# akshilpatel/tile-match-gym

Measured on AMD Instinct MI355X. Metric: env-steps/sec (whole node), 65536×10×10 boards, at 1/2/4/8 MI355X, higher is better.
Workload: dtype int8; 1 GPU; c2: 65536 x 10x10 boards per GPU, 4 colours, no specials, num_moves=30, autoreset, 3 episode-phase blocks offset by 10 steps, the timed window opening on a block's reset step (phases + 4); boards_per_gpu=65536, rows=10, cols=10, colours=4, env_groups_per_gpu=3, phase_blocks=3, policy=uniform, api=raw, graph=False, parallelism=dp1 (independent env shards, no collective)

## Files before the change

### tile-match-gym_amd/csrc/tmg_board.hip

```cpp
#include <hip/hip_runtime.h>
#include <stdint.h>

#include "pcg64.h"

namespace tmg {

#define WSYNC() __syncthreads()

#ifndef TMG_LEAN128_WAVES
#define TMG_LEAN128_WAVES 8
#endif
constexpr int kLean128Waves = TMG_LEAN128_WAVES;
constexpr int kLean128GenericWaves = 7;
constexpr int kGen128Waves = 5;
#ifndef TMG_RESET512_WAVES
#define TMG_RESET512_WAVES 8
#endif
#ifndef TMG_RESET128_WAVES
#define TMG_RESET128_WAVES 8
#endif
constexpr int kReset512Waves = TMG_RESET512_WAVES;
constexpr int kReset128Waves = TMG_RESET128_WAVES;
constexpr int kC5StepWaves = 4;

#define WFENCE() __builtin_amdgcn_fence(__ATOMIC_SEQ_CST, "wavefront")

#ifndef TMG_SMEM_DECL
#define TMG_SMEM_DECL(name) extern __shared__ __align__(16) unsigned char name[]
#endif

enum : int { SP_COOKIE = 1, SP_VLASER = 2, SP_HLASER = 4, SP_BOMB = 8 };
enum : int { M_NORMAL = 0, M_VLASER = 1, M_HLASER = 2, M_BOMB = 3, M_COOKIE = 4 };
enum : int { FL_DONE = 1, FL_COMBO = 2, FL_SHUF = 4, FL_RESET = 8, FL_OVF = 0x40, FL_ERR = 0x80 };
enum : int { TIER_MAIN = 0, TIER_SPILL = 2 };
enum : uint32_t { ST_INTERNAL = 1, ST_OVERFLOW = 2, ST_CALLER = 4 };

constexpr int kMaxShuffles = 1 << 12;

constexpr int kSpillWaves = 16;
struct SpillQ {
    uint32_t count, done;
    unsigned long long total;
    int64_t cap;
    int64_t env[1];
};

#ifndef TMG_COVER
#define TMG_COVER 0
#endif
enum : int {
    CV_SB_LEAN = 0,
    CV_SB_NORMAL,
    CV_SB_LASER,
    CV_SB_PERP_BOMB,
    CV_SB_ROW_BOMB,
    CV_SB_CLOSURE,
    CV_SB_FALLBACK,
    CV_LDS_NORMAL,
    CV_LDS_LASER,
    CV_LDS_BOMB,
    CV_LDS_FALLBACK,
    CV_SERIAL_STEP,
    CV_SERIAL_ACT,
    CV_SERIAL_COOKIE,
    CV_COMBO,
    CV_SPILL,
    CV_SPILL_RUN,
    CV_SHUFFLE,
    CV_REJECT,
    CV_FAST,
    CV_SHUFFLE_GEN,
    CV_REJECT_GEN,
    CV_RP_PASSES,
    CV_RP_PERP,
    CV_RP_VLONG,
    CV_RP_WIDE,
    CV_RP_REJECT,
    CV_LANE_STEP,
    CV_LANE_SHUFFLE,
    CV_LANE_REDRAW,
    CV_LANE_REJECT,
    CV_LANE_REJECT_REDRAW,
    CV_COUNT = 32
};
#if TMG_COVER
#define COVER(site)                                                                                     \
    do {                                                                                                \
        if (lane == 0 && P.cover) atomicAdd(P.cover + (site), 1ULL);                                   \
    } while (0)
#define COVER_L0(site)                                                                                  \
    do {                                                                                                \
        if (P.cover) atomicAdd(P.cover + (site), 1ULL);                                                \
    } while (0)
#else
#define COVER(site) ((void)0)
#define COVER_L0(site) ((void)0)
#endif

struct Params {
    int R, C, N, A, W, k, smask, num_moves;
    uint32_t thr;
    uint32_t cmag, cm1mag;
    const uint64_t *jump;
    uint64_t sb_nl[2];
    uint64_t sb_nf[2];
    uint64_t sb_h[2];
    uint64_t sb_z;
    uint64_t sb_in[2], sb_u[2], sb_v[2];
    const uint64_t *sb_rows;
    uint32_t *status;
    void *oh;
    int oh_dtype, oh_ch, oh_nsel;
    uint32_t oh_sel;
    SpillQ *spill;
    void *spill_ws;
    unsigned long long *cover;
    uint8_t *vo_term;
    uint8_t *vo_mask;
    int64_t *vo_left;
    int8_t *vo_final;
    int32_t *vo_obs;
    int sample;
    int32_t pol_t;
    int64_t pol_first;
    uint64_t pol_key;
};

#ifndef TMG_KERNARG_PARAMS
#if defined(__HIP_DEVICE_COMPILE__)
#define TMG_KERNARG_PARAMS(p) (*(const Params *)__builtin_amdgcn_kernarg_segment_ptr())
#else
#define TMG_KERNARG_PARAMS(p) (p)
#endif
#endif

inline void build_sb_rows(int R, int C, uint64_t *tab) {
    for (int r = 0; r < R; r++) {
        uint64_t m[4] = {0, 0, 0, 0};
        for (int p = 0; p < (r + 1) * C && p < 128; p++) {
            if (p >= r * C) m[p & 1] |= 1ULL << (p >> 1);
            m[2 + (p & 1)] |= 1ULL << (p >> 1);
        }
        for (int i = 0; i < 4; i++) tab[r * 4 + i] = m[i];
    }
}

inline Params make_params(int R, int C, int k, int smask, int num_moves, const uint64_t *jump) {
    Params P;
    P.R = R; P.C = C; P.N = R * C;
    P.A = 2 * R * C - R - C;
    P.W = (P.A + 63) / 64;
    P.k = k; P.smask = smask; P.num_moves = num_moves;
    const uint32_t rng = (uint32_t)(k - 1), excl = rng + 1;
    P.thr = rng ? (UINT32_MAX - rng) % excl : 0u;
    P.cmag = ((1u << 20) + (uint32_t)C - 1) / (uint32_t)C;
    P.cm1mag = C > 1 ? ((1u << 20) + (uint32_t)C - 2) / (uint32_t)(C - 1) : 0u;
    P.jump = jump;
    for (int w = 0; w < 2; w++) P.sb_nl[w] = P.sb_nf[w] = P.sb_h[w] = P.sb_in[w] = P.sb_u[w] = P.sb_v[w] = 0;
    P.sb_z = 0;
    P.sb_rows = nullptr;
    P.status = nullptr;
    P.spill = nullptr;
    P.spill_ws = nullptr;
    P.cover = nullptr;
    P.oh = nullptr;
    P.oh_dtype = P.oh_ch = P.oh_nsel = 0;
    P.oh_sel = 0;
    P.vo_term = nullptr;
    P.vo_mask = nullptr;
    P.vo_left = nullptr;
    P.vo_final = nullptr;
    P.vo_obs = nullptr;
    P.sample = 0;
    P.pol_t = 0;
    P.pol_first = 0;
    P.pol_key = 0;
    if (P.N <= 128) {
        for (int p = 0; p < P.N; p++) {
            const int c = p % C, w = p & 1, b = p >> 1;
            P.sb_in[w] |= 1ULL << b;
            if (p >= C) P.sb_u[w] |= 1ULL << b;
            if (p >= 2 * C) P.sb_v[w] |= 1ULL << b;
            if (c <= C - 2) P.sb_nl[w] |= 1ULL << b;
            if (c >= 1) P.sb_nf[w] |= 1ULL << b;
            if (c <= C - 3) P.sb_h[w] |= 1ULL << b;
        }
        const int stride = (C & 1) ? C : C / 2;
        for (int b = 0; b < 64; b += stride) P.sb_z |= 1ULL << b;
    }
    return P;
}

__device__ __forceinline__ int div_c(const Params &P, int x) { return (int)(((uint32_t)x * P.cmag) >> 20); }
__device__ __forceinline__ int div_cm1(const Params &P, int x) { return (int)(((uint32_t)x * P.cm1mag) >> 20); }


__device__ __forceinline__ int64_t wg_env() {
    const int64_t per = gridDim.x >> 3;
    return (int64_t)(blockIdx.x & 7) * per + (blockIdx.x >> 3);
}

enum : int { SC_NACT = 0, SC_NNEW, SC_ERR, SC_NZ, SC_A, SC_B, SC_C, SC_D, SC_COUNT = 16 };

template <int MAXN_>
struct WsCore {
    static constexpr int MAXN = MAXN_;
    static constexpr int NP = MAXN / 64;
    static constexpr int MAXW = (2 * MAXN) / 64 + 2;
    uint64_t effw[MAXW];
    int32_t sc[SC_COUNT];
    static constexpr int PRE = MAXW * 8 + SC_COUNT * 4;
    int8_t lpad[PRE >= 128 ? 1 : 128 - PRE];
    alignas(4) int8_t brd[2 * MAXN];
    uint8_t mark[MAXN];
    alignas(8) int8_t trash[4 * 64];
    union alignas(16) {
        uint32_t draw[MAXN + 128];
        struct { int8_t tmp[2 * MAXN]; int16_t perm[MAXN]; } sh;
    } u;
};

template <int POOL_, int MLINES_, int MQ_, int MM_, int MPOOL_, int MSTK_>
struct ListStore {
    static constexpr int POOL = POOL_;
    static constexpr int MLINES = MLINES_;
    static constexpr int MQ = MQ_;
    static constexpr int MM = MM_;
    static constexpr int MPOOL = MPOOL_;
    static constexpr int MSTK = MSTK_;
    static constexpr int MV = 96;
    int16_t pool[POOL];
    int16_t ls[MLINES], ll[MLINES];
    int16_t q[MQ];
    int16_t mpool[MPOOL];
    int16_t ms[MM], mlen[MM];
    int8_t mname[MM], mcol[MM];
// ... 1731 lines not shown
            activate(r * C + c, 2, true);
            activate(r * C + c, 3, true);
        } else if ((t1 == 4 && t2 >= 2 && t2 <= 3) || (t2 == 4 && t1 >= 2 && t1 <= 3)) {
            clr(p1); clr(p2);
            int r = r1 < r2 ? r1 : r2, c = c1 < c2 ? c1 : c2;
            int a0 = r > 0 ? r - 1 : 0, a1 = r < R - 1 ? r + 1 : R - 1;
            int b0 = c > 0 ? c - 1 : 0, b1 = c < C - 1 ? c + 1 : C - 1;
            for (int i = a0; i <= a1; i++) activate(i * C + c, 3, true);
            for (int j = b0; j <= b1; j++) activate(r * C + j, 2, true);
        } else if (t1 == 4 && t2 == 4) {
            clr(p1); clr(p2);
            int r = r1 < r2 ? r1 : r2, c = c1 < c2 ? c1 : c2;
            int a0 = r > 1 ? r - 2 : 0, a1 = r < R - 2 ? r + 2 : R - 1;
            int b0 = c > 1 ? c - 2 : 0, b1 = c < C - 2 ? c + 2 : C - 1;
            for (int i = a0; i <= a1; i++)
                for (int j = b0; j <= b1; j++) {
                    int p = i * C + j, t = typ[p];
                    if (t == 1) clr(p);
                    else if (t != 0) activate(p, t, true);
                }
        }
    }
};


#include "tmg_sb.hip"

template <int MAXN, bool GEN, int SBNB, bool CODD, int TIER, class WS, class L>
__device__ __forceinline__ int board_move(const Params &P, WS &w, int lane, const LaneJump &J, Rng &g,
                          const Cells<MAXN / 64> &cl, int p1, int p2, int &flags, int &nn, int &na, int64_t e,
                          L *lists, bool clean) {
    const auto cells = [&]() {
        if constexpr (MAXN > 128) return cl;
        else return make_cells<MAXN / 64>(P, loop_lane(lane));
    };
    const int N = P.N;
    int lim = P.R - 1;
    if (clean) lim = min(P.R - 1, div_c(P, max(p1, p2)) + 2);
    int8_t *col = w.brd, *typ = w.brd + N;
    int elim = 0;
    if (lane == 0) {
        int8_t x = col[p1]; col[p1] = col[p2]; col[p2] = x;
        x = typ[p1]; typ[p1] = typ[p2]; typ[p2] = x;
        w.sc[SC_NACT] = 0; w.sc[SC_NNEW] = 0; w.sc[SC_ERR] = 0; w.sc[SC_A] = 0;
    }
    WSYNC();
    const int t1 = typ[p1], t2 = typ[p2];
    bool ovf = false, err = false;
    if (((t1 != 0 && t1 != 1) && (t2 != 0 && t2 != 1)) || t1 < 0 || t2 < 0) {
        flags |= FL_COMBO;
        if constexpr (GEN) {
            COVER(CV_COMBO);
            int nz = count_colour_nonzero(P, w, lane);
            if (lane == 0) {
                w.sc[SC_NZ] = nz;
                Serial<MAXN, L> S(P, w, *lists);
                S.combination(p1, p2);
                w.sc[SC_A] = S.ovf;
            }
            WSYNC();
            ovf |= w.sc[SC_A] != 0;
            elim += count_type_zero(P, w, lane);
            gravity(P, w, lane);
            WSYNC();
            refill(P, w, lane, J, g);
            lim = P.R - 1;
        } else {
            err = true;
        }
    }
    bool fast = !GEN;
    if (GEN && P.smask == 0) {
        bool ok = true;
        for (int p = lane; p < N; p += 64) ok &= typ[p] == 1;
        fast = __ballot(!ok) == 0ULL;
    }
    bool plain = false;
    if constexpr (GEN && SBNB == 0) plain = !fast && !ovf && !err && plain_board(P, w, lane);
    int iters = 0;
    (void)e;
    while (!ovf && !err) {
        if (w.sc[SC_ERR]) break;
        if constexpr (GEN && SBNB > 0) {
            if (!fast) {
                const int r = sb_simple_step<SBNB, CODD>(P, w, lane, J, g);
                if (r < 0) break;
                if (r > 0) { elim += r; iters++; lim = P.R - 1; continue; }
                COVER(CV_SB_FALLBACK);
            }
        }
        Det<MAXN / 64> d;
        const int rs = detect(P, w, lane, cells(), d, lim);
        if (rs < 0) break;
        lim = P.R - 1;
        if (fast) {
            COVER(CV_FAST);
            elim += fast_clear(P, w, lane, cells(), d, rs);
            lim = min(P.R - 1, rs + 2);
        } else {
            if constexpr (GEN && SBNB == 0) {
                uint64_t cols = 0;
                int rows = 0;
                const int r = plain ? simple_step_lds(P, w, lane, d, rs, cols, rows) : 0;
                if (r > 0) {
                    elim += r;
                    gravity(P, w, lane, cols);
                    WSYNC();
                    refill(P, w, lane, J, g, rows);
                    iters++;
                    lim = min(P.R - 1, rs + 2);
                    continue;
                }
                if (plain) COVER(CV_LDS_FALLBACK);
            }
            if constexpr (GEN) {
                int nz = count_colour_nonzero(P, w, lane);
                COVER(CV_SERIAL_STEP);
                if (lane == 0) {
                    w.sc[SC_NZ] = nz;
                    Serial<MAXN, L> S(P, w, *lists);
                    S.build_lines(rs);
                    if (!S.ovf) S.process_lines();
                    if (!S.ovf) S.resolve();
                    w.sc[SC_A] = S.ovf;
                }
                WSYNC();
                ovf |= w.sc[SC_A] != 0;
                elim += count_type_zero(P, w, lane);
            }
        }
        gravity(P, w, lane);
        WSYNC();
        refill(P, w, lane, J, g);
        iters++;
    }
    (void)iters;
    nn = w.sc[SC_NNEW];
    na = w.sc[SC_NACT];
    elim += nn;
    if (ovf) flags |= FL_OVF;
    if (err || w.sc[SC_ERR]) flags |= FL_ERR;
    flags |= ensure_playable(P, w, lane, J, g, cells(), !ovf && !err && !w.sc[SC_ERR]);
    return elim;
}

__device__ __forceinline__ LaneJump load_jump(const Params &P, int lane, const Rng &g) {
    const uint64_t *t = P.jump + lane * 4;
    LaneJump J;
    J.Aj = U128{t[0], t[1]};
    J.Gj = U128{t[2], t[3]};
    J.incG = mul128(U128{g.ilo, g.ihi}, J.Gj);
    return J;
}

__device__ __forceinline__ Rng load_rng(const uint64_t *p) {
    Rng g;
    g.slo = bcast64(p[0]); g.shi = bcast64(p[1]); g.ilo = bcast64(p[2]); g.ihi = bcast64(p[3]); g.h = bcast64(p[4]);
    return g;
}
__device__ __forceinline__ void store_rng(uint64_t *p, const Rng &g, int lane) {
    if (lane == 0) { p[0] = g.slo; p[1] = g.shi; p[2] = g.ilo; p[3] = g.ihi; p[4] = g.h; }
}

#include "tmg_rp.hip"

template <int MAXN, bool GEN, int SBNB, bool CODD, int TIER = TIER_MAIN, class WS = Ws<MAXN, GEN>,
          class L = WsSerial<MAXN>>
__device__ __forceinline__ uint32_t step_env(
    const Params &P, WS &w, int lane, int64_t e, int8_t *__restrict__ board, uint64_t *__restrict__ rng, int32_t *__restrict__ timer,
    const int32_t *__restrict__ actions, int32_t *__restrict__ reward, int32_t *__restrict__ n_new,
    int32_t *__restrict__ n_act, uint8_t *__restrict__ flags_out, uint64_t *__restrict__ eff, int trust_eff,
    int autoreset, L *lists) {
    const int N = P.N, W = P.W;
    constexpr bool INLINE_GEN = !GEN && MAXN == 128;
    const bool same = autoreset == 1 || autoreset == 2;
    const bool regen_inline = autoreset == 1 || autoreset == 3;
    int a = __builtin_amdgcn_readfirstlane(actions[e]);
    const int t0 = __builtin_amdgcn_readfirstlane(timer[e]);
    const uint64_t effrow = lane < W ? eff[e * W + lane] : 0ULL;
    TMG_KEEP_V(effrow);
    if (P.sample) {
        a = __builtin_amdgcn_readfirstlane(sample_action(P, effrow, e, lane));
        if (lane == 0) const_cast<int32_t *>(actions)[e] = a;
    }
#ifndef TMG_QEXIT
#define TMG_QEXIT 1
#endif
    if (TMG_QEXIT && trust_eff && t0 < P.num_moves - 1 && (unsigned)a < (unsigned)P.A) {
        if (!((rdlane64(effrow, a >> 6) >> (a & 63)) & 1ULL)) {
            if (lane == 0) {
                uint64_t ve = (uint64_t)e;
                TMG_OPAQUE_V(ve);
                timer[ve] = t0 + 1;
                reward[ve] = 0; n_new[ve] = 0; n_act[ve] = 0;
                flags_out[ve] = (uint8_t)0;
                if (P.vo_term) reinterpret_cast<uint32_t *>(P.vo_term)[ve] = 0u;
                if (P.vo_left) P.vo_left[ve] = (int64_t)(P.num_moves - 1 - t0);
            }
            return 0;
        }
    }
    bool pend = false;
    if (t0 >= P.num_moves || a < 0 || a >= P.A) {
        pend = autoreset >= 3 && t0 >= P.num_moves;
    }
    if (!pend && (t0 >= P.num_moves || a < 0 || a >= P.A)) {
        if (lane == 0) {
            reward[e] = 0; n_new[e] = 0; n_act[e] = 0; flags_out[e] = FL_ERR;
            store_vo(P, e, FL_ERR, t0);
        }
        if ((P.oh || P.vo_obs) && !trust_eff) {
            load_board(P, w, lane, board + e * 2 * N);
            WSYNC();
            if (P.oh) store_onehot(P, w, lane, e);
            if (P.vo_obs) store_obs(P, w, lane, e);
        }
        return ST_CALLER;
    }
    int8_t *gb = board + e * 2 * N;
    uint64_t *ge = eff + e * W;
    const int t1 = t0 + 1;
    const bool done = !pend && t1 == P.num_moves;
    const bool regen = pend || (done && same);
    int flags = done ? FL_DONE : 0;
    bool effective = false;
    if (trust_eff && !pend) {
        effective = (rdlane64(effrow, a >> 6) >> (a & 63)) & 1ULL;
    }
    if (trust_eff && !effective && !(regen && regen_inline)) {
        const bool defer = regen;
        if (done && !same) {
            for (int i = lane; i < W; i += 64) ge[i] = 0ULL;
            if (P.vo_mask) store_mask(P, w, lane, e, true);
        }
        if (done && same && P.vo_final) {
            const int nbw = ((2 * N) & 3) == 0 ? (2 * N) >> 2 : 0;
            const uint32_t *src = reinterpret_cast<const uint32_t *>(gb);
            uint32_t *dst = reinterpret_cast<uint32_t *>(P.vo_final + e * 2 * N);
            for (int i = lane; i < nbw; i += 64) dst[i] = src[i];
            for (int i = 4 * nbw + lane; i < 2 * N; i += 64) P.vo_final[e * 2 * N + i] = gb[i];
        }
        if (lane == 0) {
            const int tn = defer ? 0 : t1;
            timer[e] = tn; reward[e] = 0; n_new[e] = 0; n_act[e] = 0;
            flags_out[e] = (uint8_t)(flags | (defer ? FL_RESET : 0));
            store_vo(P, e, flags, tn);
        }
        return 0;
    }
    int r1, c1, r2, c2;
    action_coords(P.R, P.C, a, r1, c1, r2, c2);
    const int p1 = r1 * P.C + c1, p2 = r2 * P.C + c2;

    const int nbw = (2 * N) >> 2;
    const bool bwhole = ((2 * N) & 3) == 0 && nbw <= 64;
    const uint32_t bw = bwhole ? reinterpret_cast<const uint32_t *>(gb)[lane < nbw ? lane : 0] : 0u;
    const uint64_t *rp = rng + e * 5;
    const uint64_t q0 = rp[0], q1 = rp[1], q2 = rp[2], q3 = rp[3], q4 = rp[4];
    constexpr bool RP = SBNB > 0 && !GEN;
    bool rowp = false;
    if constexpr (RP) rowp = rp_shape(P);
    const uint64_t *jt = P.jump + (rowp ? bp_out(lane) : lane) * 4;
    const uint64_t j0 = jt[0], j1 = jt[1], j2 = jt[2], j3 = jt[3];
    if (bwhole) {
        if (lane < nbw) reinterpret_cast<uint32_t *>(w.brd)[lane] = bw;
    } else {
        load_board(P, w, lane, gb);
    }
    if constexpr (GEN) {
        for (int p = lane; p < N; p += 64) w.mark[p] = 0;
    }
    if constexpr (TIER == TIER_SPILL) COVER(CV_SPILL_RUN);
    WSYNC();
    if constexpr (!GEN) {
        bool ok = true;
        for (int p = lane; p < N; p += 64) ok &= w.brd[N + p] == 1;
        if (__ballot(!ok) != 0ULL) {
            if (lane == 0) {
                reward[e] = 0; n_new[e] = 0; n_act[e] = 0; flags_out[e] = FL_ERR;
                store_vo(P, e, FL_ERR, t0);
            }
            return ST_INTERNAL;
        }
    }
    if (!trust_eff && !pend) {
        bool ex = lane == 0 ? eff_exact(P, w.brd, a) : false;
        effective = __ballot(ex) != 0ULL;
    }
    Rng g;
    g.slo = bcast64(q0); g.shi = bcast64(q1); g.ilo = bcast64(q2); g.ihi = bcast64(q3); g.h = bcast64(q4);
    LaneJump J;
    J.Aj = U128{j0, j1};
    J.Gj = U128{j2, j3};
    J.incG = mul128(U128{g.ilo, g.ihi}, J.Gj);
    const Cells<MAXN / 64> cl = make_cells<MAXN / 64>(P, lane);
    int elim = 0, nn = 0, na = 0;
    bool changed = false;
    if (effective) {
        if constexpr (RP) {
            if (rowp) elim = rp_move<SBNB, CODD>(P, w, lane, J, g, cl, p1, p2, flags);
            else elim = sb_move<SBNB, CODD>(P, w, lane, J, g, cl, p1, p2, flags, e);
        } else elim = board_move<MAXN, GEN, SBNB, CODD, TIER>(P, w, lane, J, g, cl, p1, p2, flags, nn, na, e, lists,
                                                             trust_eff != 0);
        changed = true;
        if constexpr (GEN) {
            if (flags & FL_OVF) {
// ... 239 lines not shown
```

### tile-match-gym_amd/csrc/tmg_rp.hip

```cpp
#ifndef TMG_RP
#define TMG_RP 1
#endif
constexpr int kRpMaxR = 16;
__device__ __forceinline__ bool rp_shape(const Params &P) {
    return TMG_RP != 0 && P.R <= kRpMaxR && P.C <= kRowScanMaxC;
}

template <int N>
__device__ __forceinline__ uint32_t rp_dn(uint32_t v, uint32_t old) {
    return (uint32_t)__builtin_amdgcn_update_dpp((int)old, (int)v, 0x110 + N, 0xf, 0xf, false);
}
template <int N>
__device__ __forceinline__ uint32_t rp_up(uint32_t v, uint32_t old) {
    return (uint32_t)__builtin_amdgcn_update_dpp((int)old, (int)v, 0x100 + N, 0xf, 0xf, false);
}
__device__ __forceinline__ uint32_t rp_or_below(uint32_t v) {
    v |= rp_up<1>(v, 0u);
    v |= rp_up<2>(v, 0u);
    v |= rp_up<4>(v, 0u);
    v |= rp_up<8>(v, 0u);
    return v;
}
__device__ __forceinline__ uint32_t rp_and_below(uint32_t v) {
    v &= rp_up<1>(v, ~0u);
    v &= rp_up<2>(v, ~0u);
    v &= rp_up<4>(v, ~0u);
    v &= rp_up<8>(v, ~0u);
    return v;
}
__device__ __forceinline__ uint32_t rp_sum_above(uint32_t v) {
    v += rp_dn<1>(v, 0u);
    v += rp_dn<2>(v, 0u);
    v += rp_dn<4>(v, 0u);
    v += rp_dn<8>(v, 0u);
    return v;
}

template <int NB, class WS>
__device__ __forceinline__ RowPlanes<NB> rp_load(const Params &P, const WS &w, int lane, uint32_t cm) {
    const int rr = lane < P.R ? lane : 0;
    const int nd = (P.C + 3) >> 2;
    uint32_t d[8];
    lds_row(w, rr * P.C, nd, d);
    RowPlanes<NB> pl;
#pragma unroll
    for (int b = 0; b < NB; b++) pl.p[b] = 0u;
#pragma unroll
    for (int j = 0; j < 8; j++) {
        if (j < nd) {
            const uint32_t x = (d[j] | 0x80808080u) - 0x01010101u;
#pragma unroll
            for (int b = 0; b < NB; b++) pl.p[b] |= byte_bits(x, b) << (4 * j);
        }
    }
#pragma unroll
    for (int b = 0; b < NB; b++) pl.p[b] &= cm;
    return pl;
}

template <int NB, int NBV, class WS>
__device__ __forceinline__ int rp_scan_nb(const Params &P, WS &w, int lane, const RowPlanes<NB> &pl, uint32_t cm) {
    uint32_t X[NBV];
    uint32_t carry = cm;
#pragma unroll
    for (int b = 0; b < NBV; b++) {
        const uint32_t x = b < NB ? pl.p[b < NB ? b : 0] : 0u;
        X[b] = x ^ carry;
        carry &= x;
    }
    return scan_rows_core<false, NBV>(P, w, lane, lane, true, X, cm, 0u, 0u, 0u, false);
}
template <int NB, class WS>
__device__ __forceinline__ int rp_scan(const Params &P, WS &w, int lane, const RowPlanes<NB> &pl, uint32_t cm) {
    constexpr int NB1 = NB < 4 ? NB + 1 : 4;
    if (rs_planes(P.k) == NB) return rp_scan_nb<NB, NB>(P, w, lane, pl, cm);
    return rp_scan_nb<NB, NB1>(P, w, lane, pl, cm);
}

__device__ __forceinline__ uint32_t rp_slice(uint64_t lo, uint64_t hi, int s, bool wide) {
    const int sh = s & 63;
    if (!wide) return (uint32_t)(lo >> sh);
    const uint64_t w0 = s < 64 ? lo : hi, w1 = s < 64 ? hi : 0ULL;
    return (uint32_t)(w0 >> sh) | (sh > 32 ? (uint32_t)(w1 << (64 - sh)) : 0u);
}

template <int NB, class WS>
__device__ __forceinline__ void rp_refill(const Params &P, WS &w, int lane, const LaneJump &J, Rng &g, uint32_t G, int pre,
                                          int T, RowPlanes<NB> &pl) {
    const uint32_t k = (uint32_t)P.k;
#pragma unroll
    for (int b = 0; b < NB; b++) pl.p[b] &= ~G;
    if (k == 1) return;
    const int off = (int)(g.h >> 32) & 1;
    const uint64_t mbuf = (uint64_t)(uint32_t)g.h * k;
    const int need = T - off;
    const int n64 = (need + 1) >> 1;
    cover_uniform(P, lane, U128{g.slo, g.shi});
    const U128 sj = jump128(J.Aj, U128{g.slo, g.shi}, J.incG);
    const uint64_t out = xsl_rr(sj);
    const int o = bp_out(lane);
    const uint64_t m0 = (uint64_t)(uint32_t)out * k, m1 = (out >> 32) * k;
    if (P.thr != 0u) {
        const bool rbuf = off && (uint32_t)mbuf < P.thr;
        const bool rej = (o < n64 && (uint32_t)m0 < P.thr) || (2 * o + 1 < need && (uint32_t)m1 < P.thr);
        if (__ballot(rej) != 0ULL || rbuf) {
            COVER(CV_REJECT);
            COVER(CV_RP_REJECT);
            WFENCE();
            if (lane == 0) {
                Rng r = g;
                for (int i = 0; i < T; i++) w.u.draw[i] = (uint32_t)r_colour(P, r);
                g = r;
            }
            rng_bcast(g);
            WSYNC();
            int at = pre;
            for (uint32_t f = G; f; f &= f - 1u) {
                const int c = __builtin_ctz(f);
                const uint32_t code = w.u.draw[at++] - 1u;
#pragma unroll
                for (int b = 0; b < NB; b++) pl.p[b] |= ((code >> b) & 1u) << c;
            }
            WSYNC();
            return;
        }
    }
    const uint32_t c0 = (uint32_t)(m0 >> 32), c1 = (uint32_t)(m1 >> 32);
    const uint32_t n0 = (uint32_t)__builtin_amdgcn_update_dpp(0, (int)c0, 0xb1, 0xf, 0xf, true);
    const uint32_t n1 = (uint32_t)__builtin_amdgcn_update_dpp(0, (int)c1, 0xb1, 0xf, 0xf, true);
    const bool odd = lane & 1;
    const uint32_t x0 = odd ? n1 : c0, x1 = odd ? c1 : n0;
    const bool wide = T > 64;
    if (wide) COVER(CV_RP_WIDE);
    const uint32_t bcode = (uint32_t)(mbuf >> 32);
    uint32_t sl[NB];
#pragma unroll
    for (int b = 0; b < NB; b++) {
        uint64_t lo = __ballot((x0 >> b) & 1u), hi = 0ULL;
        if (wide) hi = __ballot((x1 >> b) & 1u);
        if (off) {
            hi = (hi << 1) | (lo >> 63);
            lo = (lo << 1) | ((bcode >> b) & 1u);
        }
        sl[b] = rp_slice(lo, hi, pre, wide);
    }
    for (uint32_t f = G; f;) {
        const int c = __builtin_ctz(f);
        const int len = __builtin_ctz(~(f >> c));
        const uint32_t m = (1u << len) - 1u;
#pragma unroll
        for (int b = 0; b < NB; b++) {
            pl.p[b] |= (sl[b] & m) << c;
            sl[b] >>= len;
        }
        f &= ~(m << c);
    }
    if (n64 > 0) {
        const int l = bp_lane(n64 - 1);
        g.slo = rdlane64(sj.lo, l);
        g.shi = rdlane64(sj.hi, l);
        g.h = ((uint64_t)(need & 1) << 32) | (uint32_t)rdlane64(out >> 32, l);
    } else {
        g.h = (uint32_t)g.h;
    }
}

template <int NB, bool CODD, class WS>
__device__ __forceinline__ int rp_move(const Params &P, WS &w, int lane, const LaneJump &J, Rng &g,
                                       const Cells<WS::NP> &cl, int p1, int p2, int &flags) {
    const int R = P.R, C = P.C;
    int8_t *col = w.brd;
    if (lane == 0) {
        int8_t x = col[p1]; col[p1] = col[p2]; col[p2] = x;
    }
    WSYNC();
    const uint32_t cm = lane < R ? (1u << C) - 1u : 0u;
    const uint32_t hml = C >= 3 ? cm >> 2 : 0u;
    const uint32_t vml = lane >= 2 ? cm : 0u;
    RowPlanes<NB> pl = rp_load<NB>(P, w, lane, cm);
    int elim = 0;
    for (;;) {
        uint32_t neR = 0u, neU = 0u;
#pragma unroll
        for (int b = 0; b < NB; b++) {
            const uint32_t x = pl.p[b];
            neR |= x ^ (x >> 1);
            neU |= x ^ rp_dn<1>(x, 0u);
        }
        const uint32_t eqU = ~neU;
        const uint32_t h = ~(neR | (neR >> 1)) & hml;
        const uint32_t v = eqU & rp_dn<1>(eqU, 0u) & vml;
        const uint64_t rows = __ballot((h | v) != 0u);
        if (!rows) break;
        COVER(CV_SB_LEAN);
        const int rs = 63 - __clzll(rows);
        const uint32_t vv = (uint32_t)__builtin_amdgcn_readlane((int)v, rs);
        const uint32_t hh = lane == rs ? h : 0u;
        uint32_t K = hh | (hh << 1) | (hh << 2);
        if (vv) {
            const uint32_t run = rp_up<1>(rp_and_below(lane <= rs ? eqU : ~0u), ~0u);
            const uint32_t kv = lane <= rs ? vv & run : 0u;
#if TMG_COVER
            if (__ballot(lane + 3 <= rs && kv != 0u) != 0ULL) COVER(CV_RP_VLONG);
#endif
            K |= kv;
        }
        const uint32_t eqR = ~neR & (cm >> 1);
        const uint32_t walk = cm & ~K;
        const uint32_t r1 = ((K & eqR) << 1) & walk;
        const uint32_t l1 = (K >> 1) & eqR & walk;
        const uint32_t r2 = ((r1 & eqR) << 1) & walk;
        const uint32_t l2 = (l1 >> 1) & eqR & walk;
        const uint32_t q = K & ((r2 >> 2) | (l2 << 2) | ((r1 >> 1) & (l1 << 1)));
        uint32_t clr = K;
        if (q) {
            for (uint32_t f = ((q & eqR) << 1) & walk; f; f = ((f & eqR) << 1) & walk) clr |= f;
            for (uint32_t f = (q >> 1) & eqR & walk; f; f = (f >> 1) & eqR & walk) clr |= f;
        }
#if TMG_COVER
        if (__ballot(q != 0u) != 0ULL) COVER(CV_RP_PERP);
#endif
        uint32_t E = clr, G = 0u;
        for (int pass = 0;; pass++) {
            const uint32_t M = rp_or_below(E);
#pragma unroll
            for (int b = 0; b < NB; b++) pl.p[b] = (rp_dn<1>(pl.p[b], 0u) & M) | (pl.p[b] & ~M);
            E = (rp_dn<1>(E, 0u) & M) | (E & ~M);
            G = (rp_dn<1>(G, ~0u) & M) | (G & ~M);
            if (__ballot(E != 0u) == 0ULL) break;
            if (pass == 0) COVER(CV_RP_PASSES);
        }
        const int n = __builtin_popcount(G);
        const uint32_t inc = rp_sum_above((uint32_t)n);
        const int T = __builtin_amdgcn_readlane((int)inc, kRpMaxR - 1);
        elim += T;
        rp_refill<NB>(P, w, lane, J, g, G, (int)inc - n, T, pl);
    }
    const int any = rp_scan<NB>(P, w, lane, pl, cm);
    bp_to_lds<NB>(P, w, lane, pl);
    WSYNC();
    if (!any) {
        const LaneJump Jl = load_jump(P, lane, g);
        SBC c = sb_codes_from_lds(P, w.brd, lane);
        flags |= sb_ensure<NB, CODD>(P, w, lane, Jl, g, cl, c, false, true);
    }
    return elim;
}
```

### tile-match-gym_amd/tile_match_gym_amd/_native.py

```python
from __future__ import annotations

import ctypes
import hashlib
import os

from . import _buildinfo

_HERE = os.path.dirname(os.path.abspath(__file__))
DEFAULT_LIB = os.path.join(_HERE, "_lib", "libtmg.so")
LIB_PATH = os.environ.get("TMG_LIB") or DEFAULT_LIB
EXPORTS = ("tmg_create", "tmg_create_scan", "tmg_destroy", "tmg_reset", "tmg_step", "tmg_effective",
           "tmg_num_actions", "tmg_mask_words", "tmg_last_error", "tmg_abi_version", "tmg_build_info",
           "tmg_onehot", "tmg_onehot_channels", "tmg_count_states", "tmg_sample_effective", "tmg_status",
           "tmg_viable", "tmg_spills", "tmg_step_onehot", "tmg_reset_onehot", "tmg_plan_create", "tmg_plan_config",
           "tmg_plan_step", "tmg_plan_join", "tmg_plan_destroy", "tmg_plan_capture", "tmg_graph_launch",
           "tmg_graph_destroy")
DTYPE_F32, DTYPE_U8, DTYPE_I32 = 0, 1, 2
ABI_VERSION = 4
STATUS_INTERNAL, STATUS_OVERFLOW, STATUS_CALLER = 1, 2, 4

COVER_NAMES = ("sb_lean", "sb_normal", "sb_laser", "sb_perp_bomb", "sb_row_bomb", "sb_closure", "sb_fallback",
               "lds_normal", "lds_laser", "lds_bomb", "lds_fallback", "serial_step", "serial_act", "serial_cookie",
               "combo", "spill", "spill_run", "shuffle", "reject", "fast", "shuffle_gen", "reject_gen",
               "rp_passes", "rp_perp", "rp_vlong", "rp_wide", "rp_reject",
               "lane_step", "lane_shuffle", "lane_redraw", "lane_reject", "lane_reject_redraw")

SPECIAL_BITS = {"cookie": 1, "vertical_laser": 2, "horizontal_laser": 4, "bomb": 8}
FLAG_DONE, FLAG_COMBO, FLAG_SHUFFLED, FLAG_RESET, FLAG_OVERFLOW, FLAG_ERROR = 1, 2, 4, 8, 0x40, 0x80

_libs = {}

P = ctypes.c_void_p
I = ctypes.c_int
I64 = ctypes.c_int64


class TmgError(RuntimeError):
    pass


def load(path: str = None):
    path = path or LIB_PATH
    L = _libs.get(path)
    if L is not None:
        return L
    if not os.path.exists(path):
        raise TmgError(f"{path} not found: build it with `make -C tile-match-gym_amd` "
                       "(or __graft_entry__.build()); there is no CPU fallback")
    L = ctypes.CDLL(path)
    L.tmg_create.argtypes = [ctypes.POINTER(P), I, I, I, I, ctypes.c_uint32, I]
    L.tmg_create_scan.argtypes = [ctypes.POINTER(P), I, I, I]
    L.tmg_build_info.argtypes = []
    L.tmg_build_info.restype = ctypes.c_char_p
    L.tmg_destroy.argtypes = [P]
    L.tmg_reset.argtypes = [P, I64, P, P, P, P, P, P]
    L.tmg_step.argtypes = [P, I64, P, P, P, P, P, P, P, P, P, I, I, P]
    L.tmg_effective.argtypes = [P, I64, P, P, P]
    L.tmg_num_actions.argtypes = [P]
    L.tmg_mask_words.argtypes = [P]
    L.tmg_last_error.argtypes = []
    L.tmg_last_error.restype = ctypes.c_char_p
    L.tmg_abi_version.argtypes = []
    L.tmg_onehot.argtypes = [P, I64, P, P, I, P]
    L.tmg_onehot_channels.argtypes = [P]
    L.tmg_count_states.argtypes = [I, I, I, I, ctypes.POINTER(ctypes.c_uint64), ctypes.POINTER(ctypes.c_uint64)]
    L.tmg_sample_effective.argtypes = [P, I64, P, ctypes.c_uint64, I64, ctypes.c_int32, P, P]
    L.tmg_status.argtypes = [P, ctypes.POINTER(ctypes.c_uint32), I]
    L.tmg_viable.argtypes = [I, I, I]
    L.tmg_spills.argtypes = [P, ctypes.POINTER(ctypes.c_uint64)]
    L.tmg_step_onehot.argtypes = [P, I64, P, P, P, P, P, P, P, P, P, I, I, P, I, P]
    L.tmg_reset_onehot.argtypes = [P, I64, P, P, P, P, P, P, I, P]
    L.tmg_plan_create.argtypes = [ctypes.POINTER(P), P, I64, P, P, P, P, P, P, P, P, I, P, P]
    L.tmg_plan_config.argtypes = [P, I, I, ctypes.c_uint64, I64, P, I, P, P, P, P, P]
    L.tmg_plan_step.argtypes = [P, P, ctypes.c_int32, I, I, P]
    L.tmg_plan_join.argtypes = [P, P]
    L.tmg_plan_destroy.argtypes = [P]
    L.tmg_plan_capture.argtypes = [P, I, P, P, I, P, ctypes.POINTER(P)]
    L.tmg_graph_launch.argtypes = [P, P]
    L.tmg_graph_destroy.argtypes = [P]
    for name in ("tmg_create", "tmg_create_scan", "tmg_destroy", "tmg_reset", "tmg_step", "tmg_effective",
                 "tmg_num_actions", "tmg_mask_words", "tmg_abi_version", "tmg_onehot", "tmg_onehot_channels",
                 "tmg_sample_effective", "tmg_status", "tmg_viable", "tmg_spills", "tmg_step_onehot", "tmg_reset_onehot",
                 "tmg_count_states", "tmg_plan_create", "tmg_plan_config", "tmg_plan_step", "tmg_plan_join",
                 "tmg_plan_destroy", "tmg_plan_capture", "tmg_graph_launch", "tmg_graph_destroy"):
        getattr(L, name).restype = I
    if L.tmg_abi_version() != ABI_VERSION:
        raise TmgError("libtmg.so ABI version mismatch; rebuild it")
    info = _parse_info(L.tmg_build_info().decode())
    want = _buildinfo.source_hash()
    if want is not None and info.get("src") != want:
        raise TmgError(f"{path} was built from other sources (src={info.get('src')}, tree={want}): "
                       "stale build, run `make -C tile-match-gym_amd -B`")
    if path == DEFAULT_LIB and info.get("variant") != "product":
        raise TmgError(f"{path} is a {info.get('variant')!r} build, not the product library")
    _libs[path] = L
    return L


def _parse_info(s: str) -> dict:
    return dict(kv.split("=", 1) for kv in s.split(";") if "=" in kv)


def build_info(path: str = None) -> dict:
    path = path or LIB_PATH
    L = load(path)
    info = _parse_info(L.tmg_build_info().decode())
    with open(path, "rb") as f:
        info["so_sha256"] = hashlib.sha256(f.read()).hexdigest()
    info["path"] = path
    return info


def check(rc: int, L=None):
    if rc != 0:
        msg = (L or load()).tmg_last_error().decode(errors="replace")
        raise TmgError(f"libtmg error {rc}: {msg}")


def specials_mask(colourless_specials, colour_specials) -> int:
    m = 0
    for name in list(colourless_specials) + list(colour_specials):
        if name not in SPECIAL_BITS:
            raise ValueError(f"unknown special {name!r}")
        m |= SPECIAL_BITS[name]
    return m


class Context:

    def __init__(self, device_index: int, rows: int, cols: int, colours: int = 0, smask: int = 0,
                 num_moves: int = 1, scan_only: bool = False, lib_path: str = None):
        L = self._L = load(lib_path)
        h = P()
        if scan_only:
            check(L.tmg_create_scan(ctypes.byref(h), int(device_index), int(rows), int(cols)), L)
        else:
            check(L.tmg_create(ctypes.byref(h), int(device_index), int(rows), int(cols), int(colours),
                               int(smask), int(num_moves)), L)
        self._h = h
        self.num_actions = L.tmg_num_actions(h)
        self.mask_words = L.tmg_mask_words(h)

    def _check(self, rc: int):
        check(rc, self._L)

    @property
    def handle(self):
        return self._h

    def close(self):
        if getattr(self, "_h", None) is not None and self._h.value:
            self._L.tmg_destroy(self._h)
            self._h = None

    def __del__(self):
        try:
            self.close()
        except Exception:
            pass

    def reset(self, n, board, rng, timer, eff, env_mask, stream, onehot=None, onehot_dtype=DTYPE_F32):
        if onehot:
            self._check(self._L.tmg_reset_onehot(self._h, int(n), board, rng, timer, eff, env_mask, onehot,
                                          int(onehot_dtype), stream))
        else:
            self._check(self._L.tmg_reset(self._h, int(n), board, rng, timer, eff, env_mask, stream))

    def step(self, n, board, rng, timer, actions, reward, n_new, n_act, flags, eff, trust_eff, autoreset, stream,
             onehot=None, onehot_dtype=DTYPE_F32):
        if onehot:
            self._check(self._L.tmg_step_onehot(self._h, int(n), board, rng, timer, actions, reward, n_new, n_act, flags,
                                         eff, int(trust_eff), int(autoreset), onehot, int(onehot_dtype), stream))
        else:
            self._check(self._L.tmg_step(self._h, int(n), board, rng, timer, actions, reward, n_new, n_act, flags, eff,
                                  int(trust_eff), int(autoreset), stream))

    def status(self, clear: bool = False) -> int:
        v = ctypes.c_uint32(0)
        self._check(self._L.tmg_status(self._h, ctypes.byref(v), int(clear)))
        return int(v.value)

    def spills(self) -> int:
        v = ctypes.c_uint64(0)
        self._check(self._L.tmg_spills(self._h, ctypes.byref(v)))
        return int(v.value)

    def effective(self, n, board, eff, stream):
        self._check(self._L.tmg_effective(self._h, int(n), board, eff, stream))

    def onehot_channels(self) -> int:
        return self._L.tmg_onehot_channels(self._h)

    def onehot(self, n, board, out, out_dtype, stream):
        self._check(self._L.tmg_onehot(self._h, int(n), board, out, int(out_dtype), stream))

    def cover(self, clear: bool = False):
        L = self._L
        fn = getattr(L, "tmg_debug_cover", None)
        if fn is None:
            raise TmgError("this context's library is not a TMG_COVER build")
        import numpy as np
        out = np.zeros(32, np.uint64)
        fn.argtypes = [P, P, I, I]
        fn.restype = I
        check(fn(self._h, out.ctypes.data, 32, int(clear)), L)
        return out

    def sample_effective(self, n, eff, key, first_env, t, actions, stream):
        self._check(self._L.tmg_sample_effective(self._h, int(n), eff, int(key) & 0xFFFFFFFFFFFFFFFF, int(first_env),
                                          int(t), actions, stream))


class Plan:

    AUTORESET = {"none": 0, "same_step": 1, "next_step": 2}

    def __init__(self, ctx: "Context", n, board, rng, timer, reward, n_new, n_act, flags, eff, bounds, streams):
        L = self._L = ctx._L
        self._ctx = ctx
        G = len(streams)
        self._bounds = (ctypes.c_int64 * (G + 1))(*[int(b) for b in bounds])
        self._streams = (P * G)(*[int(x) for x in streams])
        h = P()
        check(L.tmg_plan_create(ctypes.byref(h), ctx.handle, int(n), board, rng, timer, reward, n_new, n_act, flags,
                                eff, G, self._bounds, self._streams), L)
        self._h = h
        self._step = L.tmg_plan_step
        self._join = L.tmg_plan_join

    def config(self, autoreset="same_step", policy=False, key=0, first_env=0, onehot=None, onehot_dtype=DTYPE_F32,
               terminated=None, action_mask=None, moves_left=None, final_board=None, board32=None):
        check(self._L.tmg_plan_config(self._h, self.AUTORESET[autoreset], int(bool(policy)),
                                      int(key) & 0xFFFFFFFFFFFFFFFF, int(first_env), onehot, int(onehot_dtype),
                                      terminated, action_mask, moves_left, final_board, board32), self._L)

    def step(self, actions_ptr: int, t: int, trust_eff: int, stream: int, fork: int = 1):
        rc = self._step(self._h, actions_ptr, t, trust_eff, fork, stream)
        if rc:
            check(rc, self._L)

    def join(self, stream: int):
        rc = self._join(self._h, stream)
        if rc:
            check(rc, self._L)

    def capture(self, actions_ptrs, ts, trust_eff: int, stream: int) -> "StepGraph":
        k = len(actions_ptrs)
        a = (P * k)(*[int(x) for x in actions_ptrs])
        t = (ctypes.c_int32 * k)(*[int(x) for x in ts])
        h = P()
        check(self._L.tmg_plan_capture(self._h, k, a, t, int(trust_eff), stream, ctypes.byref(h)), self._L)
        return StepGraph(self, h, k)

    def close(self):
        if getattr(self, "_h", None) is not None and self._h.value:
            self._L.tmg_plan_destroy(self._h)
            self._h = None

    def __del__(self):
        try:
            self.close()
        except Exception:
            pass


class StepGraph:

    def __init__(self, plan: Plan, h, steps: int):
        self._plan, self._h, self.steps = plan, h, steps
        self._L = plan._L

    def launch(self, stream: int):
        rc = self._L.tmg_graph_launch(self._h, stream)
        if rc:
            check(rc, self._L)

    def close(self):
        if getattr(self, "_h", None) is not None and self._h.value:
            self._L.tmg_graph_destroy(self._h)
            self._h = None

    def __del__(self):
        try:
            self.close()
        except Exception:
            pass


_SCAN_CTX = {}


def scan_context(device_index: int, rows: int, cols: int) -> "Context":
    key = (int(device_index), int(rows), int(cols))
    c = _SCAN_CTX.get(key)
    if c is None:
        c = _SCAN_CTX[key] = Context(key[0], key[1], key[2], scan_only=True)
    return c


def viable(rows: int, cols: int, colours: int) -> bool:
    return bool(load().tmg_viable(int(rows), int(cols), int(colours)))


def count_states(device_index: int, rows: int, cols: int, colours: int):
    a, b = ctypes.c_uint64(0), ctypes.c_uint64(0)
    check(load().tmg_count_states(int(device_index), int(rows), int(cols), int(colours), ctypes.byref(a),
                                  ctypes.byref(b)))
    return int(a.value), int(b.value)
```

Measured before the change: 1.183 billion env-steps/s.

## Batch RNG colour draws across cascade passes in row-plane move

```diff
diff --git a/tile-match-gym_amd/csrc/tmg_board.hip b/tile-match-gym_amd/csrc/tmg_board.hip
--- a/tile-match-gym_amd/csrc/tmg_board.hip
+++ b/tile-match-gym_amd/csrc/tmg_board.hip
@@ -81,7 +81,9 @@
     CV_LANE_REDRAW,
     CV_LANE_REJECT,
     CV_LANE_REJECT_REDRAW,
-    CV_COUNT = 32
+    CV_RP_CARRY,
+    CV_RP_REBATCH,
+    CV_COUNT = 40
 };
 #if TMG_COVER
 #define COVER(site)                                                                                     \
@@ -2119,6 +2121,9 @@
     J.incG = mul128(U128{g.ilo, g.ihi}, J.Gj);
     return J;
 }
+__device__ __forceinline__ LaneJump load_jump_bp(const Params &P, int lane, const Rng &g) {
+    return load_jump(P, bp_out(lane), g);
+}
 
 __device__ __forceinline__ Rng load_rng(const uint64_t *p) {
     Rng g;
diff --git a/tile-match-gym_amd/csrc/tmg_rp.hip b/tile-match-gym_amd/csrc/tmg_rp.hip
--- a/tile-match-gym_amd/csrc/tmg_rp.hip
+++ b/tile-match-gym_amd/csrc/tmg_rp.hip
@@ -84,6 +84,49 @@
     return (uint32_t)(w0 >> sh) | (sh > 32 ? (uint32_t)(w1 << (64 - sh)) : 0u);
 }
 
+#ifndef TMG_RP_BATCH
+#define TMG_RP_BATCH 1
+#endif
+
+template <int NB, class WS>
+__device__ __forceinline__ void rp_replay(const Params &P, WS &w, int lane, Rng &g, uint32_t G, int pre, int T,
+                                          RowPlanes<NB> &pl) {
+    COVER(CV_REJECT);
+    COVER(CV_RP_REJECT);
+    WFENCE();
+    if (lane == 0) {
+        Rng r = g;
+        for (int i = 0; i < T; i++) w.u.draw[i] = (uint32_t)r_colour(P, r);
+        g = r;
+    }
+    rng_bcast(g);
+    WSYNC();
+    int at = pre;
+    for (uint32_t f = G; f; f &= f - 1u) {
+        const int c = __builtin_ctz(f);
+        const uint32_t code = w.u.draw[at++] - 1u;
+#pragma unroll
+        for (int b = 0; b < NB; b++) pl.p[b] |= ((code >> b) & 1u) << c;
+    }
+    WSYNC();
+}
+
+template <int NB>
+__device__ __forceinline__ void rp_deposit(uint32_t G, uint32_t (&sl)[NB], RowPlanes<NB> &pl) {
+    for (uint32_t f = G; f;) {
+        const int c = __builtin_ctz(f);
+        const int len = __builtin_ctz(~(f >> c));
+        const uint32_t m = (1u << len) - 1u;
+#pragma unroll
+        for (int b = 0; b < NB; b++) {
+            pl.p[b] |= (sl[b] & m) << c;
+            sl[b] >>= len;
+        }
+        f &= ~(m << c);
+    }
+}
+
+#if !TMG_RP_BATCH
 template <int NB, class WS>
 __device__ __forceinline__ void rp_refill(const Params &P, WS &w, int lane, const LaneJump &J, Rng &g, uint32_t G, int pre,
                                           int T, RowPlanes<NB> &pl) {
@@ -104,24 +147,7 @@
         const bool rbuf = off && (uint32_t)mbuf < P.thr;
         const bool rej = (o < n64 && (uint32_t)m0 < P.thr) || (2 * o + 1 < need && (uint32_t)m1 < P.thr);
         if (__ballot(rej) != 0ULL || rbuf) {
-            COVER(CV_REJECT);
-            COVER(CV_RP_REJECT);
-            WFENCE();
-            if (lane == 0) {
-                Rng r = g;
-                for (int i = 0; i < T; i++) w.u.draw[i] = (uint32_t)r_colour(P, r);
-                g = r;
-            }
-            rng_bcast(g);
-            WSYNC();
-            int at = pre;
-            for (uint32_t f = G; f; f &= f - 1u) {
-                const int c = __builtin_ctz(f);
-                const uint32_t code = w.u.draw[at++] - 1u;
-#pragma unroll
-                for (int b = 0; b < NB; b++) pl.p[b] |= ((code >> b) & 1u) << c;
-            }
-            WSYNC();
+            rp_replay<NB>(P, w, lane, g, G, pre, T, pl);
             return;
         }
     }
@@ -144,17 +170,7 @@
         }
         sl[b] = rp_slice(lo, hi, pre, wide);
     }
-    for (uint32_t f = G; f;) {
-        const int c = __builtin_ctz(f);
-        const int len = __builtin_ctz(~(f >> c));
-        const uint32_t m = (1u << len) - 1u;
-#pragma unroll
-        for (int b = 0; b < NB; b++) {
-            pl.p[b] |= (sl[b] & m) << c;
-            sl[b] >>= len;
-        }
-        f &= ~(m << c);
-    }
+    rp_deposit<NB>(G, sl, pl);
     if (n64 > 0) {
         const int l = bp_lane(n64 - 1);
         g.slo = rdlane64(sj.lo, l);
@@ -164,12 +180,134 @@
         g.h = (uint32_t)g.h;
     }
 }
+#else
+template <int NB>
+struct RpBatch {
+    U128 sj;
+    uint64_t lo[NB], hi[NB];
+    int rfirst;
+    int left;
+    int used;
+    int off;
+};
+
+template <int NB>
+__device__ __forceinline__ void rp_advance(RpBatch<NB> &B, int T) {
+    if (T < 64) {
+#pragma unroll
+        for (int b = 0; b < NB; b++) {
+            B.lo[b] = (B.lo[b] >> T) | (B.hi[b] << (64 - T));
+            B.hi[b] >>= T;
+        }
+    } else {
+#pragma unroll
+        for (int b = 0; b < NB; b++) {
+            B.lo[b] = T < 128 ? B.hi[b] >> (T - 64) : 0ULL;
+            B.hi[b] = 0ULL;
+        }
+    }
+    B.left -= T;
+    B.used += T;
+}
+
+template <int NB>
+__device__ __forceinline__ void rp_batch(const Params &P, int lane, const LaneJump &J, const Rng &g, RpBatch<NB> &B) {
+    const uint32_t k = (uint32_t)P.k;
+    const int off = (int)(g.h >> 32) & 1;
+    const uint64_t mbuf = (uint64_t)(uint32_t)g.h * k;
+    cover_uniform(P, lane, U128{g.slo, g.shi});
+    B.sj = jump128(J.Aj, U128{g.slo, g.shi}, J.incG);
+    const uint64_t out = xsl_rr(B.sj);
+    const uint64_t m0 = (uint64_t)(uint32_t)out * k, m1 = (out >> 32) * k;
+    uint32_t c0 = (uint32_t)(m0 >> 32), c1 = (uint32_t)(m1 >> 32);
+    if (P.thr != 0u) {
+        c0 |= (uint32_t)m0 < P.thr ? 0x80000000u : 0u;
+        c1 |= (uint32_t)m1 < P.thr ? 0x80000000u : 0u;
+    }
+    const uint32_t n0 = (uint32_t)__builtin_amdgcn_update_dpp(0, (int)c0, 0xb1, 0xf, 0xf, true);
+    const uint32_t n1 = (uint32_t)__builtin_amdgcn_update_dpp(0, (int)c1, 0xb1, 0xf, 0xf, true);
+    const bool odd = lane & 1;
+    const uint32_t x0 = odd ? n1 : c0, x1 = odd ? c1 : n0;
+    const uint32_t bcode = (uint32_t)(mbuf >> 32);
+#pragma unroll
+    for (int b = 0; b < NB; b++) {
+        uint64_t lo = __ballot((x0 >> b) & 1u), hi = __ballot((x1 >> b) & 1u);
+        if (off) {
+            hi = (hi << 1) | (lo >> 63);
+            lo = (lo << 1) | ((bcode >> b) & 1u);
+        }
+        B.lo[b] = lo;
+        B.hi[b] = hi;
+    }
+    B.rfirst = 2 * 128;
+    if (P.thr != 0u) {
+        const uint64_t lo = __ballot((x0 >> 31) != 0u), hi = __ballot((x1 >> 31) != 0u);
+        if (lo | hi) B.rfirst = off + (lo ? __builtin_ctzll(lo) : 64 + __builtin_ctzll(hi));
+        if (off && (uint32_t)mbuf < P.thr) B.rfirst = 0;
+    }
+    B.left = 128;
+    B.used = 0;
+    B.off = off;
+}
+
+template <int NB>
+__device__ __forceinline__ void rp_sync(RpBatch<NB> &B, Rng &g) {
+    if (B.used > 0) {
+        const int need = B.used - B.off;
+        if (need > 0) {
+            const int l = bp_lane(((need + 1) >> 1) - 1);
+            const U128 s{rdlane64(B.sj.lo, l), rdlane64(B.sj.hi, l)};
+            g.slo = s.lo;
+            g.shi = s.hi;
+            g.h = ((uint64_t)(need & 1) << 32) | (uint32_t)(xsl_rr(s) >> 32);
+        } else {
+            g.h = (uint32_t)g.h;
+        }
+    }
+    B.left = 0;
+    B.used = 0;
+}
+
+template <int NB, class WS>
+__device__ __forceinline__ void rp_take(const Params &P, WS &w, int lane, RpBatch<NB> &B, Rng &g, uint32_t G, int pre,
+                                        int T, RowPlanes<NB> &pl) {
+#pragma unroll
+    for (int b = 0; b < NB; b++) pl.p[b] &= ~G;
+    if (P.k == 1) return;
+    if (B.left < T) {
+        if (B.used > 0) COVER(CV_RP_REBATCH);
+        rp_sync(B, g);
+        const LaneJump J = load_jump_bp(P, lane, g);
+        rp_batch<NB>(P, lane, J, g, B);
+    } else if (B.used > 0) {
+        COVER(CV_RP_CARRY);
+    }
+    if (P.thr != 0u) {
+        if (B.used + T > B.rfirst) {
+            rp_sync(B, g);
+            rp_replay<NB>(P, w, lane, g, G, pre, T, pl);
+            return;
+        }
+    }
+    const bool wide = T > 64;
+    if (wide) COVER(CV_RP_WIDE);
+    uint32_t sl[NB];
+#pragma unroll
+    for (int b = 0; b < NB; b++) sl[b] = rp_slice(B.lo[b], B.hi[b], pre, wide);
+    rp_advance(B, T);
+    rp_deposit<NB>(G, sl, pl);
+}
+#endif
 
 template <int NB, bool CODD, class WS>
 __device__ __forceinline__ int rp_move(const Params &P, WS &w, int lane, const LaneJump &J, Rng &g,
                                        const Cells<WS::NP> &cl, int p1, int p2, int &flags) {
     const int R = P.R, C = P.C;
     int8_t *col = w.brd;
+#if TMG_RP_BATCH
+    RpBatch<NB> B{};
+    if (P.k != 1) rp_batch<NB>(P, lane, J, g, B);
+#endif
     if (lane == 0) {
         int8_t x = col[p1]; col[p1] = col[p2]; col[p2] = x;
     }
@@ -234,8 +372,14 @@
         const uint32_t inc = rp_sum_above((uint32_t)n);
         const int T = __builtin_amdgcn_readlane((int)inc, kRpMaxR - 1);
         elim += T;
+#if TMG_RP_BATCH
+        rp_take<NB>(P, w, lane, B, g, G, (int)inc - n, T, pl);
+    }
+    rp_sync(B, g);
+#else
         rp_refill<NB>(P, w, lane, J, g, G, (int)inc - n, T, pl);
     }
+#endif
     const int any = rp_scan<NB>(P, w, lane, pl, cm);
     bp_to_lds<NB>(P, w, lane, pl);
     WSYNC();
diff --git a/tile-match-gym_amd/tile_match_gym_amd/_native.py b/tile-match-gym_amd/tile_match_gym_amd/_native.py
--- a/tile-match-gym_amd/tile_match_gym_amd/_native.py
+++ b/tile-match-gym_amd/tile_match_gym_amd/_native.py
@@ -23,7 +23,8 @@
                "lds_normal", "lds_laser", "lds_bomb", "lds_fallback", "serial_step", "serial_act", "serial_cookie",
                "combo", "spill", "spill_run", "shuffle", "reject", "fast", "shuffle_gen", "reject_gen",
                "rp_passes", "rp_perp", "rp_vlong", "rp_wide", "rp_reject",
-               "lane_step", "lane_shuffle", "lane_redraw", "lane_reject", "lane_reject_redraw")
+               "lane_step", "lane_shuffle", "lane_redraw", "lane_reject", "lane_reject_redraw",
+               "rp_carry", "rp_rebatch")
 
 SPECIAL_BITS = {"cookie": 1, "vertical_laser": 2, "horizontal_laser": 4, "bomb": 8}
 FLAG_DONE, FLAG_COMBO, FLAG_SHUFFLED, FLAG_RESET, FLAG_OVERFLOW, FLAG_ERROR = 1, 2, 4, 8, 0x40, 0x80
@@ -200,10 +201,10 @@
         if fn is None:
             raise TmgError("this context's library is not a TMG_COVER build")
         import numpy as np
-        out = np.zeros(32, np.uint64)
+        out = np.zeros(len(COVER_NAMES), np.uint64)
         fn.argtypes = [P, P, I, I]
         fn.restype = I
-        check(fn(self._h, out.ctypes.data, 32, int(clear)), L)
+        check(fn(self._h, out.ctypes.data, out.size, int(clear)), L)
         return out
 
     def sample_effective(self, n, eff, key, first_env, t, actions, stream):
```

Result: faster. 1.279 billion env-steps/s (median of 6 runs) (+8.1%).
